# daigo0927/tf-raft

Hardware: NVIDIA H100
Metric: frame-pairs/sec at 448×512 iters=12; final-flow max-abs vs ref (higher is better)
Workload: dtype f32

## Files before the change

tf_raft_b200/csrc/conv_tc.cuh:

```cuda
#pragma once
#include "common.cuh"
#include "kernels.cuh"
#include "tmap.cuh"

namespace raft {

enum TcEpilogue : int {
  EPI_LINEAR = 0,
  EPI_GRU_ZR = 1,
  EPI_GRU_Q = 2,
};
enum TcAct : int { ACT_NONE = 0, ACT_RELU = 1 };

constexpr int kTileM = 128;
constexpr int kChunkK = 64;
constexpr int kABytes = kTileM * kChunkK * 2;
constexpr int kMaxTileN = 128;
constexpr int kConsumerWGs = 2;
constexpr int kConsumerWarps = 4 * kConsumerWGs;
constexpr int kTcThreads = 128 * kConsumerWGs + 128;
constexpr int kStageCols = 64;
constexpr int kStagingBytes = kConsumerWGs * 64 * kStageCols * 4;
constexpr int kSmemMax = 227 * 1024;
constexpr int kSmemFixed = 1024  + kStagingBytes + 512 ;

struct alignas(64) TcConvParams {
  CUtensorMap a_map[2];
  CUtensorMap b_map;
  int nseg, seg_chunks[2], seg_c0[2];
  int kh, kw, ph, pw;
  int stride;
  int B, H, W, TH, TW, tiles_x, tiles_y;
  int bn, n_total;
  int n_tiles_n;
  int nstages, stage_bytes;
  int group_chunks;
  int mode, act;
  const float* bias;
  const float* inv_scale;
  float out_scale;
  float* out_f32; int f32_stride, f32_c0;
  __half* out_hi; __half* out_lo; int h_stride, h_c0;
  const float* post_scale;
  const float* post_shift;
  const float* residual; int res_stride, res_c0;
  const float* concat_src; int concat_n;
  float* z; int hid;
  float* h;
  float* adv_coords;
  float* adv_flow;
};

#if defined(__CUDA_ARCH__)
__device__ __forceinline__ float4 ld4(const float* p) { return *reinterpret_cast<const float4*>(p); }
__device__ __forceinline__ float4 ldg4(const float* p) { return __ldg(reinterpret_cast<const float4*>(p)); }
__device__ __forceinline__ void st4(float* p, float4 v) { *reinterpret_cast<float4*>(p) = v; }
__device__ __forceinline__ void st8u(void* p, const uint32_t (&r)[8]) {
  reinterpret_cast<uint4*>(p)[0] = make_uint4(r[0], r[1], r[2], r[3]);
  reinterpret_cast<uint4*>(p)[1] = make_uint4(r[4], r[5], r[6], r[7]);
}
__device__ __forceinline__ void ldcg8(const float* p, float (&r)[8]) {
  const float4 a = __ldcg(reinterpret_cast<const float4*>(p)), b = __ldcg(reinterpret_cast<const float4*>(p) + 1);
  r[0] = a.x; r[1] = a.y; r[2] = a.z; r[3] = a.w; r[4] = b.x; r[5] = b.y; r[6] = b.z; r[7] = b.w;
}
__device__ __forceinline__ void ldnc8(const float* p, float (&r)[8]) {
  const float4 a = __ldg(reinterpret_cast<const float4*>(p)), b = __ldg(reinterpret_cast<const float4*>(p) + 1);
  r[0] = a.x; r[1] = a.y; r[2] = a.z; r[3] = a.w; r[4] = b.x; r[5] = b.y; r[6] = b.z; r[7] = b.w;
}
__device__ __forceinline__ void st8f(float* p, float a, float b, float c, float d, float e, float f, float g, float h) {
  const uint32_t r[8] = {__float_as_uint(a), __float_as_uint(b), __float_as_uint(c), __float_as_uint(d),
                         __float_as_uint(e), __float_as_uint(f), __float_as_uint(g), __float_as_uint(h)};
  st8u(p, r);
}
__device__ __forceinline__ float4 ldcg4(const float* p) { return __ldcg(reinterpret_cast<const float4*>(p)); }

__device__ __forceinline__ float fast_sigmoid(float x) { return __fdividef(1.0f, 1.0f + __expf(-x)); }
__device__ __forceinline__ float fast_tanh(float x) { return 1.0f - __fdividef(2.0f, 1.0f + __expf(2.0f * x)); }

template <int MODE>
__device__ __forceinline__ void tc_epilogue_regs(const TcConvParams& p, float (&v)[32], size_t pix, int col, int ncol,
                                                 float inv_scale) {
  if (p.bias) {
#pragma unroll
    for (int q = 0; q < 8; ++q) {
      const float4 bq = ldg4(p.bias + col + 4 * q);
      v[4 * q] = v[4 * q] * inv_scale + bq.x; v[4 * q + 1] = v[4 * q + 1] * inv_scale + bq.y;
      v[4 * q + 2] = v[4 * q + 2] * inv_scale + bq.z; v[4 * q + 3] = v[4 * q + 3] * inv_scale + bq.w;
    }
  } else {
#pragma unroll
    for (int j = 0; j < 32; ++j) v[j] *= inv_scale;
  }
  if (MODE == EPI_LINEAR && p.post_scale) {
#pragma unroll
    for (int q = 0; q < 8; ++q) {
      const float4 sc = ldg4(p.post_scale + col + 4 * q), sh = ldg4(p.post_shift + col + 4 * q);
      v[4 * q] = v[4 * q] * sc.x + sh.x; v[4 * q + 1] = v[4 * q + 1] * sc.y + sh.y;
      v[4 * q + 2] = v[4 * q + 2] * sc.z + sh.z; v[4 * q + 3] = v[4 * q + 3] * sc.w + sh.w;
    }
  }

  __half* dhi = nullptr;
  __half* dlo = nullptr;
  if (MODE == EPI_LINEAR) {
    const bool full = col + 32 <= p.n_total;
#pragma unroll
    for (int j = 0; j < 32; ++j) {
      if (p.act == ACT_RELU) v[j] = relu_nan(v[j]);
      v[j] *= p.out_scale;
    }
    if (full) {
      if (p.residual) {
        const float* rp = p.residual + pix * (size_t)p.res_stride + p.res_c0 + col;
        if (((p.res_stride | p.res_c0) & 7) == 0) {
#pragma unroll
          for (int q = 0; q < 4; ++q) {
            float r8[8];
            ldnc8(rp + 8 * q, r8);
#pragma unroll
            for (int e = 0; e < 8; ++e) v[8 * q + e] = relu_nan(v[8 * q + e] + r8[e]);
          }
        } else if (((p.res_stride | p.res_c0) & 3) == 0) {
#pragma unroll
          for (int q = 0; q < 8; ++q) {
            const float4 r4 = ldg4(rp + 4 * q);
            v[4 * q] = relu_nan(v[4 * q] + r4.x); v[4 * q + 1] = relu_nan(v[4 * q + 1] + r4.y);
            v[4 * q + 2] = relu_nan(v[4 * q + 2] + r4.z); v[4 * q + 3] = relu_nan(v[4 * q + 3] + r4.w);
          }
        } else {
#pragma unroll
          for (int j = 0; j < 32; ++j) v[j] = relu_nan(v[j] + __ldg(rp + j));
        }
      }
    } else {
#pragma unroll
      for (int j = 0; j < 32; ++j) {
        const int cj = col + j - p.n_total;
        if (cj >= 0) v[j] = (p.concat_src && cj < p.concat_n) ? __ldg(p.concat_src + pix * p.concat_n + cj) : 0.0f;
        else if (p.residual) v[j] = relu_nan(v[j] + __ldg(p.residual + pix * (size_t)p.res_stride + p.res_c0 + col + j));
      }
    }
    if (p.out_f32) {
      const int nvalid = min(ncol, p.n_total - col);
      float* dst = p.out_f32 + pix * (size_t)p.f32_stride + p.f32_c0 + col;
      if (nvalid == 32 && ((p.f32_stride | p.f32_c0) & 7) == 0) {
#pragma unroll
        for (int q = 0; q < 4; ++q)
          st8f(dst + 8 * q, v[8 * q], v[8 * q + 1], v[8 * q + 2], v[8 * q + 3], v[8 * q + 4], v[8 * q + 5], v[8 * q + 6], v[8 * q + 7]);
      } else if (nvalid == 32 && ((p.f32_stride | p.f32_c0) & 3) == 0) {
#pragma unroll
        for (int q = 0; q < 8; ++q) st4(dst + 4 * q, make_float4(v[4 * q], v[4 * q + 1], v[4 * q + 2], v[4 * q + 3]));
      } else {
#pragma unroll
        for (int j = 0; j < 32; ++j)
          if (j < nvalid) dst[j] = v[j];
      }
    }
    if (p.out_hi && ncol == 32) {
      const size_t o = pix * (size_t)p.h_stride + p.h_c0 + col;
      dhi = p.out_hi + o;
      dlo = p.out_lo + o;
    }
    if (p.adv_coords && col == 0) {
      float2 c1 = __ldcg(reinterpret_cast<const float2*>(p.adv_coords) + pix);
      c1.x = __fadd_rn(c1.x, v[0]);
      c1.y = __fadd_rn(c1.y, v[1]);
      reinterpret_cast<float2*>(p.adv_coords)[pix] = c1;
      const float gx = (float)(pix % p.W), gy = (float)((pix / p.W) % p.H);
      reinterpret_cast<float2*>(p.adv_flow)[pix] = make_float2(__fsub_rn(c1.x, gx), __fsub_rn(c1.y, gy));
    }
  } else if (MODE == EPI_GRU_ZR) {
    if (col < p.hid) {
      float* dst = p.z + pix * (size_t)p.hid + col;
      if ((p.hid & 7) == 0) {
#pragma unroll
        for (int q = 0; q < 4; ++q)
          st8f(dst + 8 * q, fast_sigmoid(v[8 * q]), fast_sigmoid(v[8 * q + 1]), fast_sigmoid(v[8 * q + 2]), fast_sigmoid(v[8 * q + 3]),
               fast_sigmoid(v[8 * q + 4]), fast_sigmoid(v[8 * q + 5]), fast_sigmoid(v[8 * q + 6]), fast_sigmoid(v[8 * q + 7]));
      } else {
#pragma unroll
        for (int q = 0; q < 8; ++q)
          st4(dst + 4 * q, make_float4(fast_sigmoid(v[4 * q]), fast_sigmoid(v[4 * q + 1]), fast_sigmoid(v[4 * q + 2]),
                                       fast_sigmoid(v[4 * q + 3])));
      }
    } else {
      const int hc = col - p.hid;
      const float* hp = p.h + pix * (size_t)p.hid + hc;
      if ((p.hid & 7) == 0) {
#pragma unroll
        for (int q = 0; q < 4; ++q) {
          float h8[8];
          ldcg8(hp + 8 * q, h8);
#pragma unroll
          for (int e = 0; e < 8; ++e) v[8 * q + e] = fast_sigmoid(v[8 * q + e]) * h8[e];
        }
      } else {
#pragma unroll
        for (int q = 0; q < 8; ++q) {
          const float4 hv = ldcg4(hp + 4 * q);
          v[4 * q] = fast_sigmoid(v[4 * q]) * hv.x; v[4 * q + 1] = fast_sigmoid(v[4 * q + 1]) * hv.y;
          v[4 * q + 2] = fast_sigmoid(v[4 * q + 2]) * hv.z; v[4 * q + 3] = fast_sigmoid(v[4 * q + 3]) * hv.w;
        }
      }
      const size_t o = pix * (size_t)p.h_stride + p.h_c0 + hc;
      dhi = p.out_hi + o;
      dlo = p.out_lo + o;
    }
  } else if (MODE == EPI_GRU_Q) {
    float* hrow = p.h + pix * (size_t)p.hid + col;
    const float* zp = p.z + pix * (size_t)p.hid + col;
#pragma unroll
    for (int q = 0; q < 8; ++q) {
      const float4 zv = ldcg4(zp + 4 * q), hv = ldcg4(hrow + 4 * q);
      v[4 * q] = (1.0f - zv.x) * hv.x + zv.x * fast_tanh(v[4 * q]);
      v[4 * q + 1] = (1.0f - zv.y) * hv.y + zv.y * fast_tanh(v[4 * q + 1]);
      v[4 * q + 2] = (1.0f - zv.z) * hv.z + zv.z * fast_tanh(v[4 * q + 2]);
      v[4 * q + 3] = (1.0f - zv.w) * hv.w + zv.w * fast_tanh(v[4 * q + 3]);
    }
#pragma unroll
    for (int q = 0; q < 8; ++q) st4(hrow + 4 * q, make_float4(v[4 * q], v[4 * q + 1], v[4 * q + 2], v[4 * q + 3]));
    const size_t o = pix * (size_t)p.h_stride + p.h_c0 + col;
    dhi = p.out_hi + o;
    dlo = p.out_lo + o;
  }

  if (dhi) {
    const bool wide = ((reinterpret_cast<uintptr_t>(dhi) | reinterpret_cast<uintptr_t>(dlo)) & 31) == 0;
#pragma unroll
    for (int q = 0; q < 2; ++q) {
      uint32_t ph[8], pl[8];
#pragma unroll
      for (int e = 0; e < 8; ++e) split_f16x2(v[16 * q + 2 * e], v[16 * q + 2 * e + 1], ph[e], pl[e]);
      if (wide) {
        st8u(dhi + 16 * q, ph);
        st8u(dlo + 16 * q, pl);
      } else {
        reinterpret_cast<uint4*>(dhi)[2 * q] = make_uint4(ph[0], ph[1], ph[2], ph[3]);
        reinterpret_cast<uint4*>(dhi)[2 * q + 1] = make_uint4(ph[4], ph[5], ph[6], ph[7]);
        reinterpret_cast<uint4*>(dlo)[2 * q] = make_uint4(pl[0], pl[1], pl[2], pl[3]);
        reinterpret_cast<uint4*>(dlo)[2 * q + 1] = make_uint4(pl[4], pl[5], pl[6], pl[7]);
      }
    }
  }
}

struct RingPos {
  int slot;
  uint32_t par;
};

__device__ __forceinline__ int ring_next(RingPos& r, int nst) {
  const int s = r.slot;
  r.slot = s + 1 == nst ? 0 : s + 1;
  return s;
}

__device__ __forceinline__ void ring_init(uint64_t* full_bar, uint64_t* empty_bar, int nst) {
  for (int s = 0; s < nst; ++s) {
    mbar_init(&full_bar[s], 1);
    mbar_init(&empty_bar[s], kConsumerWarps);
  }
}

struct RingSlot {
  uint8_t* data;
  uint64_t* full;
};

__device__ __forceinline__ RingSlot ring_acquire(uint8_t* stages, const int& slot_bytes, const int& nst, uint64_t* full_bar,
                                                 uint64_t* empty_bar, RingPos& rp, const int& tx) {
  const int s = ring_next(rp, nst);
  mbar_wait(&empty_bar[s], ((rp.par >> s) & 1u) ^ 1u);
  rp.par ^= 1u << s;
  mbar_arrive_expect_tx(&full_bar[s], (uint32_t)tx);
  return RingSlot{stages + (size_t)s * slot_bytes, &full_bar[s]};
}

template <int N>
__device__ __forceinline__ void ring_mma(float (&racc)[N / 2], uint8_t* stages, const int& slot_bytes, const int& nst,
                                         uint64_t* full_bar, uint64_t* empty_bar, RingPos& rp, int wg, uint32_t b_lo_off,
                                         int total, const int& group_chunks) {
  const int lane = threadIdx.x & 31;
  float acc[N / 2];
#pragma unroll
  for (int i = 0; i < N / 2; ++i) acc[i] = racc[i] = 0.0f;
  for (int done = 0; done < total;) {
    const int gend = min(total, done + group_chunks);
    for (int first = 1; done < gend; ++done, first = 0) {
      const int s = ring_next(rp, nst);
      mbar_wait(&full_bar[s], (rp.par >> s) & 1u);
      rp.par ^= 1u << s;
      const uint32_t sa = smem_u32(stages + (size_t)s * slot_bytes);
      const uint32_t arow = (uint32_t)wg * 64 * 128;
      wgmma_fence_regs(acc);
      wgmma_fence();
      wgmma_chunk3<N>(acc, make_desc_sw128(sa + arow), make_desc_sw128(sa + kABytes + arow), make_desc_sw128(sa + 2 * kABytes),
                      make_desc_sw128(sa + 2 * kABytes + b_lo_off), first != 0);
      wgmma_commit();
      wgmma_wait_all();
      wgmma_fence_regs(acc);
      __syncwarp();
      if (lane == 0) mbar_arrive(&empty_bar[s]);
    }
#pragma unroll
    for (int i = 0; i < N / 2; ++i) racc[i] += acc[i];
  }
}

__device__ __forceinline__ int tc_total_chunks(const TcConvParams& c) {
  return c.kh * c.kw * (c.seg_chunks[0] + (c.nseg > 1 ? c.seg_chunks[1] : 0));
}

__device__ __forceinline__ void tc_produce_tile(const TcConvParams& c, uint8_t* stages, uint64_t* full_bar, uint64_t* empty_bar,
                                                RingPos& rp, int nt, int b, int ty, int tx, unsigned int* next_item = nullptr,
                                                int* claim = nullptr) {
  const int ntaps = c.kh * c.kw;
  const int x0 = tx * c.TW * c.stride, y0 = ty * c.TH * c.stride, n0 = nt * c.bn;
  int left = tc_total_chunks(c);
  for (int tap = 0; tap < ntaps; ++tap) {
    const int dy = tap / c.kw - c.ph, dx = tap % c.kw - c.pw;
    int kc = 0;
    for (int seg = 0; seg < c.nseg; ++seg) {
      for (int ch = 0; ch < c.seg_chunks[seg]; ++ch, ++kc) {
        if (--left == 0 && claim) *claim = (int)atomicAdd(next_item, 1u);
        const RingSlot st = ring_acquire(stages, c.stage_bytes, c.nstages, full_bar, empty_bar, rp, c.stage_bytes);
        tma_load_5d(st.data, &c.a_map[seg], st.full, c.seg_c0[seg] + ch * kChunkK, x0 + dx, y0 + dy, b, 0);
        tma_load_4d(st.data + 2 * kABytes, &c.b_map, st.full, kc * kChunkK, n0, tap, 0);
      }
    }
  }
}

__device__ __forceinline__ int stg_idx(int r, int c) { return r * kStageCols + ((((c >> 2) ^ (r & 7))) << 2) + (c & 3); }

template <int N>
__device__ __forceinline__ void tc_consume_tile(const TcConvParams& c, uint8_t* stages, float* staging, uint64_t* full_bar,
                                                uint64_t* empty_bar, RingPos& rp, int wg, int tid, int nt, int b, int ty,
                                                int tx) {
  const int lane = tid & 31, w = tid >> 5;
  float racc[N / 2];
  ring_mma<N>(racc, stages, c.stage_bytes, c.nstages, full_bar, empty_bar, rp, wg, (uint32_t)(c.bn * kChunkK * 2),
              tc_total_chunks(c), c.group_chunks);

  float* stg = staging + wg * 64 * kStageCols;
  const int row = tid & 63, half = tid >> 6;
  const int m = wg * 64 + row;
  const int x = tx * c.TW + m % c.TW, y = ty * c.TH + m / c.TW;
  const bool inside = x < c.W && y < c.H;
  const size_t pix = ((size_t)b * c.H + y) * c.W + x;
  const float inv_scale = c.inv_scale ? __ldg(c.inv_scale) : 1.0f;
#pragma unroll
  for (int cb = 0; cb < (N + kStageCols - 1) / kStageCols; ++cb) {
    if (cb * kStageCols >= c.bn) break;
    wg_sync(wg);
#pragma unroll
    for (int i = cb * 8; i < min(cb * 8 + 8, N / 8); ++i) {
      const int col = 8 * (i - cb * 8) + 2 * (lane & 3), r0 = 16 * w + (lane >> 2);
      *reinterpret_cast<float2*>(stg + stg_idx(r0, col)) = make_float2(racc[4 * i], racc[4 * i + 1]);
      *reinterpret_cast<float2*>(stg + stg_idx(r0 + 8, col)) = make_float2(racc[4 * i + 2], racc[4 * i + 3]);
    }
    wg_sync(wg);
    const int c0 = cb * kStageCols + half * 32;
    if (inside && c0 < c.bn) {
      const int ncol = min(32, c.bn - c0);
      float v[32];
#pragma unroll
      for (int q = 0; q < 8; ++q) {
        const float4 t4 = *reinterpret_cast<const float4*>(stg + stg_idx(row, half * 32 + 4 * q));
        v[4 * q] = t4.x; v[4 * q + 1] = t4.y; v[4 * q + 2] = t4.z; v[4 * q + 3] = t4.w;
      }
#pragma unroll
      for (int j = 0; j < 32; ++j)
        if (j >= ncol) v[j] = 0.0f;
      if (c.mode == EPI_LINEAR) tc_epilogue_regs<EPI_LINEAR>(c, v, pix, nt * c.bn + c0, ncol, inv_scale);
      else if (c.mode == EPI_GRU_ZR) tc_epilogue_regs<EPI_GRU_ZR>(c, v, pix, nt * c.bn + c0, ncol, inv_scale);
      else tc_epilogue_regs<EPI_GRU_Q>(c, v, pix, nt * c.bn + c0, ncol, inv_scale);
    }
  }
}

template <class F>
__device__ __forceinline__ void with_mma_n(int bn, F&& f) {
  if (bn <= 16) f(std::integral_constant<int, 16>{});
  else if (bn <= 32) f(std::integral_constant<int, 32>{});
  else if (bn <= 64) f(std::integral_constant<int, 64>{});
  else if (bn <= 96) f(std::integral_constant<int, 96>{});
  else f(std::integral_constant<int, 128>{});
}

__device__ __forceinline__ void regs_producer() { asm volatile("setmaxnreg.dec.sync.aligned.u32 40;\n" ::: "memory"); }
__device__ __forceinline__ void regs_consumer() { asm volatile("setmaxnreg.inc.sync.aligned.u32 232;\n" ::: "memory"); }

__device__ __forceinline__ void tc_decode_tile(const TcConvParams& c, int t, int& nt, int& b, int& ty, int& tx) {
  const int mtiles = c.B * c.tiles_y * c.tiles_x;
  nt = t / mtiles;
  int mt = t - nt * mtiles;
  tx = mt % c.tiles_x;
  mt /= c.tiles_x;
  ty = mt % c.tiles_y;
  b = mt / c.tiles_y;
}
#endif

__global__ void __launch_bounds__(kTcThreads, 1) conv_tc_kernel(const __grid_constant__ TcConvParams p) {
#if defined(__CUDA_ARCH__)
  extern __shared__ uint8_t smem_raw[];
  uint8_t* smem = reinterpret_cast<uint8_t*>((reinterpret_cast<uintptr_t>(smem_raw) + 1023) & ~uintptr_t(1023));
  const int nst = p.nstages;
  uint8_t* stages = smem;
  float* staging = reinterpret_cast<float*>(stages + (size_t)nst * p.stage_bytes);
  uint64_t* full_bar = reinterpret_cast<uint64_t*>(reinterpret_cast<uint8_t*>(staging) + kStagingBytes);
  uint64_t* empty_bar = full_bar + nst;

  const int warp = threadIdx.x >> 5;
  const int mtiles = p.B * p.tiles_y * p.tiles_x;
  const int ntiles = mtiles * p.n_tiles_n;

  if (threadIdx.x == 0) {
    ring_init(full_bar, empty_bar, nst);
    fence_mbar_init();
  }
  if (warp == kConsumerWarps && (threadIdx.x & 31) == 0) {
    prefetch_tmap(&p.a_map[0]);
    prefetch_tmap(&p.b_map);
    if (p.nseg > 1) prefetch_tmap(&p.a_map[1]);
  }
  __syncthreads();
  asm volatile("griddepcontrol.wait;" ::: "memory");
  asm volatile("griddepcontrol.launch_dependents;" ::: "memory");

  RingPos rp{0, 0u};
  if (warp >= kConsumerWarps) {
    regs_producer();
    if (warp == kConsumerWarps && elect_one()) {
      for (int t = blockIdx.x; t < ntiles; t += gridDim.x) {
        int nt, b, ty, tx;
        tc_decode_tile(p, t, nt, b, ty, tx);
        tc_produce_tile(p, stages, full_bar, empty_bar, rp, nt, b, ty, tx);
      }
    }
  } else {
    regs_consumer();
    const int wg = warp >> 2, tid = threadIdx.x & 127;
    with_mma_n(p.bn, [&](auto n) {
      for (int t = blockIdx.x; t < ntiles; t += gridDim.x) {
        int nt, b, ty, tx;
        tc_decode_tile(p, t, nt, b, ty, tx);
        tc_consume_tile<decltype(n)::value>(p, stages, staging, full_bar, empty_bar, rp, wg, tid, nt, b, ty, tx);
      }
    });
  }
#endif
}

inline void tc_pick_tile(int W, int H, int* tw, int* th) {
  long best = -1;
  for (int t = 128; t >= 8; t >>= 1) {
    const int hh = 128 / t;
    const long area = (long)round_up(W, t) * round_up(H, hh);
    if (best < 0 || area < best) {
      best = area;
      *tw = t;
      *th = hh;
    }
  }
}

inline int tc_n_split(int bn) {
  const int f = ceil_div(bn, kMaxTileN);
  return bn % (16 * f) == 0 ? f : 0;
}

inline int tc_finalize(TcConvParams& p) {
  p.tiles_x = ceil_div(p.W, p.TW);
  p.tiles_y = ceil_div(p.H, p.TH);
  p.stage_bytes = 2 * kABytes + 2 * p.bn * kChunkK * 2;
  int nst = (kSmemMax - kSmemFixed) / p.stage_bytes;
  if (nst > 8) nst = 8;
  p.nstages = nst;
  return nst * p.stage_bytes + kSmemFixed;
}

inline int tc_check(const TcConvParams& p) {
  if (p.bn % 16 != 0 || p.bn < 16 || p.bn > kMaxTileN || p.TW * p.TH != kTileM) return RAFT_ERR_BAD_SHAPE;
  if (p.mode != EPI_LINEAR && p.mode != EPI_GRU_ZR && p.mode != EPI_GRU_Q) return RAFT_ERR_UNSUPPORTED;
  if (p.group_chunks < 1) return RAFT_ERR_BAD_ARG;
  return RAFT_OK;
}

template <auto Kernel>
inline int persistent_grid(int smem, long items, unsigned* grid) {
  static int num_sms[64] = {0};
  int dev = 0;
  RAFT_CUDA_TRY(cudaGetDevice(&dev));
  int& sms = num_sms[dev & 63];
  if (!sms) {
    RAFT_CUDA_TRY(cudaFuncSetAttribute(Kernel, cudaFuncAttributeMaxDynamicSharedMemorySize, smem));
    RAFT_CUDA_TRY(cudaDeviceGetAttribute(&sms, cudaDevAttrMultiProcessorCount, dev));
  }
  *grid = (unsigned)(items < sms ? items : sms);
  return RAFT_OK;
}

inline int tc_launch(TcConvParams& p, int n_tiles_n, cudaStream_t stream) {
  RAFT_TRY(tc_check(p));
  if (p.stride < 1) p.stride = 1;
  const int smem = tc_finalize(p);
  if (p.nstages < 2) return RAFT_ERR_UNSUPPORTED;
  p.n_tiles_n = n_tiles_n;
  unsigned grid = 0;
  RAFT_TRY(persistent_grid<conv_tc_kernel>(kSmemMax, (long)p.B * p.tiles_y * p.tiles_x * n_tiles_n, &grid));
  cudaLaunchConfig_t cfg;
  memset(&cfg, 0, sizeof(cfg));
  cfg.gridDim = dim3(grid);
  cfg.blockDim = dim3((unsigned)kTcThreads);
  cfg.dynamicSmemBytes = (size_t)smem;
  cfg.stream = stream;
  cudaLaunchAttribute attr[1];
  attr[0].id = cudaLaunchAttributeProgrammaticStreamSerialization;
  attr[0].val.programmaticStreamSerializationAllowed = 1;
  cfg.attrs = attr;
  cfg.numAttrs = 1;
  ++g_launches;
  RAFT_CUDA_TRY(cudaLaunchKernelEx(&cfg, conv_tc_kernel, p));
  return raft_launch_status();
}

struct TcWeightSlot {
  size_t hi, lo, bias, scale, absmax;
  int kh, kw, cin_pad, cout_pad;
};

inline TcWeightSlot tc_weight_slot(size_t& off, int kh, int kw, int cin_pad, int cout_pad) {
  auto take = [&](size_t bytes) { const size_t o = off; off = align_up(off + bytes, 256); return o; };
  TcWeightSlot s;
  s.kh = kh; s.kw = kw; s.cin_pad = cin_pad; s.cout_pad = cout_pad;
  const size_t plane = (size_t)kh * kw * cout_pad * cin_pad * sizeof(__half);
  s.hi = take(plane);
  s.lo = take(plane);
  s.bias = take(sizeof(float) * (cout_pad + 64));
  s.scale = take(2 * sizeof(float));
  s.absmax = take(sizeof(unsigned int));
  return s;
}

struct TcCinMap { int nrange, src0[2], n[2], dst0[2]; };

inline int tc_pack_weights(uint8_t* base, const TcWeightSlot& s, const raft_conv* const src[], int nsrc,
                           const TcCinMap* cin_map, bool flatten, cudaStream_t st) {
  unsigned int* amax = reinterpret_cast<unsigned int*>(base + s.absmax);
  float* scale = reinterpret_cast<float*>(base + s.scale);
  for (int i = 0; i < nsrc; ++i) {
    const size_t nw = (size_t)src[i]->kh * src[i]->kw * src[i]->cin * src[i]->cout;
    RAFT_TRY(launch(absmax_kernel, grid_for(nw), 256, 0, st, src[i]->kernel, nw, amax));
  }
  RAFT_TRY(launch(weight_scale_kernel, 1, 1, 0, st, amax, scale));
  int cout_off = 0;
  for (int i = 0; i < nsrc; ++i) {
    const raft_conv& cv = *src[i];
    PackParams pp;
    memset(&pp, 0, sizeof(pp));
    pp.w = cv.kernel;
    pp.kh = cv.kh; pp.kw = cv.kw; pp.cin = cv.cin; pp.cout = cv.cout;
    if (flatten) { pp.cin = pp.kh * pp.kw * pp.cin; pp.kh = pp.kw = 1; }
    pp.hi = reinterpret_cast<__half*>(base + s.hi);
    pp.lo = reinterpret_cast<__half*>(base + s.lo);
    pp.cout_pad = s.cout_pad; pp.cin_pad = s.cin_pad; pp.cout_off = cout_off;
    const TcCinMap m = cin_map ? *cin_map : TcCinMap{1, {0, 0}, {pp.cin, 0}, {0, 0}};
    pp.nrange = m.nrange;
    for (int r = 0; r < m.nrange; ++r) {
      pp.r_src0[r] = m.src0[r];
      pp.r_n[r] = m.n[r];
      pp.r_dst0[r] = m.dst0[r];
    }
    pp.scale = scale;
    RAFT_TRY(launch(pack_weights_kernel, grid_for((size_t)cv.kh * cv.kw * cv.cin * cv.cout), 256, 0, st, pp));
    RAFT_CUDA_TRY(cudaMemcpyAsync(base + s.bias + cout_off * sizeof(float), cv.bias, cv.cout * sizeof(float),
                                  cudaMemcpyDeviceToDevice, st));
    cout_off += cv.cout;
  }
  return RAFT_OK;
}

inline int tc_use_weights(TcConvParams& p, const uint8_t* base, const TcWeightSlot& s, int bn) {
  RAFT_TRY(make_tmap_wgt2(&p.b_map, reinterpret_cast<const __half*>(base + s.hi),
                          reinterpret_cast<const __half*>(base + s.lo), s.kh * s.kw, s.cout_pad, s.cin_pad, bn));
  p.kh = s.kh; p.kw = s.kw;
  p.bn = bn;
  p.bias = reinterpret_cast<const float*>(base + s.bias);
  p.inv_scale = reinterpret_cast<const float*>(base + s.scale) + 1;
  return RAFT_OK;
}

}
```

tf_raft_b200/csrc/encoder.cuh:

```cuda
#pragma once
#include <algorithm>

#include "lookup.cuh"
#include "update.cuh"

namespace raft {

enum { NORM_NONE = 0, NORM_INSTANCE = 1, NORM_BATCH = 2 };

struct EncSpec { int c0; int c[3]; int s[3]; };
inline EncSpec enc_spec(int variant) {
  if (variant == RAFT_VARIANT_BASIC) return {64, {64, 96, 128}, {1, 2, 2}};
  return {32, {32, 64, 96}, {1, 2, 2}};
}
inline int pad64(int c) { return round_up(c, 64); }

struct EncNormSlot { size_t gamma, beta, fscale, fshift; int C; };
struct EncLayout {
  TcWeightSlot conv1;
  EncNormSlot norm1;
  TcWeightSlot bc1[6], bc2[6], bds[6];
  EncNormSlot bn1[6], bn2[6], bnd[6];
  int has_ds[6], bc[6], bstride[6];
  TcWeightSlot conv2;
  size_t total;
};

inline EncLayout enc_layout(int variant, int out_dim) {
  EncLayout L;
  memset(&L, 0, sizeof(L));
  const EncSpec S = enc_spec(variant);
  size_t off = 0;
  auto take = [&](size_t bytes) { size_t o = off; off = align_up(off + bytes, 256); return o; };
  auto conv_slot = [&](int kh, int kw, int cin, int cout) { return tc_weight_slot(off, kh, kw, pad64(cin), round_up(cout, 32)); };
  auto norm_slot = [&](int C) {
    EncNormSlot n;
    n.C = C;
    n.gamma = take(sizeof(float) * (C + 64)); n.beta = take(sizeof(float) * (C + 64));
    n.fscale = take(sizeof(float) * (C + 64)); n.fshift = take(sizeof(float) * (C + 64));
    return n;
  };
  L.conv1 = conv_slot(1, 1, 147, S.c0);
  L.norm1 = norm_slot(S.c0);
  int cin = S.c0;
  for (int k = 0; k < 6; ++k) {
    const int c = S.c[k / 2], st = (k % 2 == 0) ? S.s[k / 2] : 1;
    L.bc[k] = c; L.bstride[k] = st;
    L.bc1[k] = conv_slot(3, 3, cin, c);
    L.bc2[k] = conv_slot(3, 3, c, c);
    L.bn1[k] = norm_slot(c);
    L.bn2[k] = norm_slot(c);
    L.has_ds[k] = st != 1;
    if (L.has_ds[k]) { L.bds[k] = conv_slot(1, 1, cin, c); L.bnd[k] = norm_slot(c); }
    cin = c;
  }
  L.conv2 = conv_slot(1, 1, cin, out_dim);
  L.total = off;
  return L;
}

struct EncWs {
  float *X32, *O32, *Y32, *D32;
  __half *Xh, *Xl, *Oh, *Ol, *Fh, *Fl, *Ih, *Il;
  float *part, *mean, *mult;
  size_t total;
};
constexpr int kNormSplit = 64;
inline EncWs enc_ws_layout(void* base, int variant, int N, int H, int W) {
  EncWs E;
  memset(&E, 0, sizeof(E));
  const EncSpec S = enc_spec(variant);
  size_t max32 = 0, max16 = 0;
  for (int l = 0; l < 3; ++l) {
    const int d = 2 << l;
    const size_t np = (size_t)N * ((H + d - 1) / d) * ((W + d - 1) / d);
    const int c = l == 0 ? (S.c0 > S.c[0] ? S.c0 : S.c[0]) : S.c[l];
    if (np * c > max32) max32 = np * c;
    if (np * pad64(c) > max16) max16 = np * pad64(c);
  }
  uint8_t* b8 = reinterpret_cast<uint8_t*>(base);
  size_t off = 0;
  auto take = [&](size_t bytes) { uint8_t* p = b8 + off; off = align_up(off + bytes, 1024); return p; };
  E.X32 = (float*)take(max32 * 4); E.O32 = (float*)take(max32 * 4);
  E.Y32 = (float*)take(max32 * 4); E.D32 = (float*)take(max32 * 4);
  E.Xh = (__half*)take(max16 * 2); E.Xl = (__half*)take(max16 * 2);
  E.Oh = (__half*)take(max16 * 2); E.Ol = (__half*)take(max16 * 2);
  E.Fh = (__half*)take(max16 * 2); E.Fl = (__half*)take(max16 * 2);
  {
    const size_t np1 = (size_t)N * ((H + 1) / 2) * ((W + 1) / 2);
    E.Ih = (__half*)take(np1 * 192 * 2); E.Il = (__half*)take(np1 * 192 * 2);
  }
  E.part = (float*)take((size_t)N * kNormSplit * 3 * 256 * 4);
  E.mean = (float*)take((size_t)N * 256 * 4);
  E.mult = (float*)take((size_t)N * 256 * 4);
  E.total = off;
  return E;
}

inline int enc_pack_conv(const raft_conv& cv, int kh, int kw, int cin, int cout, const TcWeightSlot& s, bool flatten,
                         uint8_t* base, cudaStream_t st) {
  if (!cv.kernel || !cv.bias) return RAFT_ERR_BAD_ARG;
  if (cv.kh != kh || cv.kw != kw || cv.cin != cin || cv.cout != cout) return RAFT_ERR_BAD_SHAPE;
  const raft_conv* src[1] = {&cv};
  return tc_pack_weights(base, s, src, 1, nullptr, flatten, st);
}

inline int enc_pack_norm(const raft_norm& nm, const EncNormSlot& s, int norm_type, uint8_t* base, cudaStream_t st) {
  if (norm_type == NORM_NONE) return 0;
  if (!nm.gamma || !nm.beta) return RAFT_ERR_BAD_ARG;
  float* g = reinterpret_cast<float*>(base + s.gamma);
  float* b = reinterpret_cast<float*>(base + s.beta);
  RAFT_CUDA_TRY(cudaMemcpyAsync(g, nm.gamma, s.C * sizeof(float), cudaMemcpyDeviceToDevice, st));
  RAFT_CUDA_TRY(cudaMemcpyAsync(b, nm.beta, s.C * sizeof(float), cudaMemcpyDeviceToDevice, st));
  if (norm_type == NORM_BATCH) {
    if (!nm.moving_mean || !nm.moving_variance) return RAFT_ERR_BAD_ARG;
    return launch(bn_fold_kernel, ceil_div(s.C, 128), 128, 0, st, nm.gamma, nm.beta, nm.moving_mean, nm.moving_variance,
                  1e-3f, s.C, reinterpret_cast<float*>(base + s.fscale), reinterpret_cast<float*>(base + s.fshift));
  }
  return raft_launch_status();
}

inline int encoder_prepare(int variant, int norm_type, int out_dim, const raft_encoder_weights* w, void* prepared,
                           size_t bytes, cudaStream_t st) {
  const EncLayout L = enc_layout(variant, out_dim);
  if (L.total > bytes) return RAFT_ERR_WORKSPACE;
  const EncSpec S = enc_spec(variant);
  uint8_t* base = reinterpret_cast<uint8_t*>(prepared);
  RAFT_CUDA_TRY(cudaMemsetAsync(base, 0, L.total, st));
  RAFT_TRY(enc_pack_conv(w->conv1, 7, 7, 3, S.c0, L.conv1, true, base, st));
  RAFT_TRY(enc_pack_norm(w->norm1, L.norm1, norm_type, base, st));
  int cin = S.c0;
  for (int k = 0; k < 6; ++k) {
    const int c = L.bc[k];
    RAFT_TRY(enc_pack_conv(w->block[k].conv1, 3, 3, cin, c, L.bc1[k], false, base, st));
    RAFT_TRY(enc_pack_conv(w->block[k].conv2, 3, 3, c, c, L.bc2[k], false, base, st));
    RAFT_TRY(enc_pack_norm(w->block[k].norm1, L.bn1[k], norm_type, base, st));
    RAFT_TRY(enc_pack_norm(w->block[k].norm2, L.bn2[k], norm_type, base, st));
    if (L.has_ds[k]) {
      RAFT_TRY(enc_pack_conv(w->block[k].downsample, 1, 1, cin, c, L.bds[k], false, base, st));
      RAFT_TRY(enc_pack_norm(w->block[k].downsample_norm, L.bnd[k], norm_type, base, st));
    }
    cin = c;
  }
  RAFT_TRY(enc_pack_conv(w->conv2, 1, 1, cin, out_dim, L.conv2, false, base, st));
  return raft_launch_status();
}

struct EncCtx {
  const uint8_t* prep; EncLayout L; EncWs W; cudaStream_t st;
  int N, norm_type, stats;
  int per_image;
};

inline int enc_norm_apply(const EncCtx& c, const EncNormSlot& ns, const float* y, size_t npix, int P, int relu,
                          const float* skip32, const __half* skip_hi, const __half* skip_lo, float* out32, __half* hi,
                          __half* lo) {
  const int C = ns.C, G = c.per_image ? c.N : 1;
  const int Pg = c.per_image ? P : (int)npix;
  const float* gamma = reinterpret_cast<const float*>(c.prep + ns.gamma);
  const float* beta = reinterpret_cast<const float*>(c.prep + ns.beta);
  RAFT_TRY(launch(norm_stats_kernel, dim3((unsigned)G, kNormSplit), 256, 0, c.st, y, Pg, C, kNormSplit, c.W.part));
  RAFT_TRY(launch(norm_final_kernel, ceil_div(G * C * 32, 256), 256, 0, c.st, c.W.part, G, C, kNormSplit, gamma, 1e-3f,
                  c.W.mean, c.W.mult));
  return launch(norm_apply_kernel, grid_for(npix * (pad64(C) / 8)), 256, 0, c.st, y, npix, P, C, c.per_image, c.W.mean,
                c.W.mult, beta, relu, skip32, skip_hi, skip_lo, out32, hi, lo, pad64(C));
}

inline int enc_conv_tc(const EncCtx& c, const TcWeightSlot& cs, int cout, const EncNormSlot* ns, const __half* ahi,
                       const __half* alo, int Hin, int Win, int Hout, int Wout, int stride, int relu, const float* skip,
                       float* out32, __half* ohi, __half* olo) {
  TcConvParams p;
  memset(&p, 0, sizeof(p));
  int tw, th;
  tc_pick_tile(Wout, Hout, &tw, &th);
  if (tw * stride > 256) tw = 128 / stride, th = 128 / tw;
  const int nsplit = tc_n_split(cs.cout_pad);
  if (!nsplit) return RAFT_ERR_BAD_SHAPE;
  RAFT_TRY(make_tmap_act2(&p.a_map[0], ahi, alo, c.N, Hin, Win, cs.cin_pad, tw, th, stride));
  RAFT_TRY(tc_use_weights(p, c.prep, cs, cs.cout_pad / nsplit));
  p.nseg = 1; p.seg_chunks[0] = cs.cin_pad / kChunkK; p.seg_c0[0] = 0;
  p.stride = stride;
  if (stride == 1) { p.ph = (cs.kh - 1) / 2; p.pw = (cs.kw - 1) / 2; }
  else {
    const int tot_h = (Hout - 1) * stride + cs.kh - Hin, tot_w = (Wout - 1) * stride + cs.kw - Win;
    p.ph = (tot_h > 0 ? tot_h : 0) / 2; p.pw = (tot_w > 0 ? tot_w : 0) / 2;
  }
  p.B = c.N; p.H = Hout; p.W = Wout; p.TH = th; p.TW = tw;
  p.n_total = cout;
  p.mode = EPI_LINEAR; p.out_scale = 1.0f;
  p.out_f32 = out32; p.f32_stride = cout; p.f32_c0 = 0;
  p.out_hi = ohi; p.out_lo = olo; p.h_stride = pad64(cout); p.h_c0 = 0;
  if (ns && !c.stats && c.norm_type == NORM_BATCH) {
    p.post_scale = reinterpret_cast<const float*>(c.prep + ns->fscale);
    p.post_shift = reinterpret_cast<const float*>(c.prep + ns->fshift);
  }
  const bool fused = !(ns && c.stats);
  if (fused) {
    p.act = relu ? ACT_RELU : ACT_NONE;
    p.residual = skip; p.res_stride = cout; p.res_c0 = 0;
  } else {
    p.act = ACT_NONE; p.out_hi = nullptr; p.out_lo = nullptr;
  }
  p.group_chunks = 5;
  return tc_launch(p, nsplit, c.st);
}

inline int encoder_forward(int variant, int norm_type, int out_dim, const void* prepared, const float* images, int N,
                           int H, int W, int training, int image_norm, float* out, void* ws, size_t ws_bytes, cudaStream_t st) {
  EncCtx c;
  c.prep = reinterpret_cast<const uint8_t*>(prepared);
  c.L = enc_layout(variant, out_dim);
  c.W = enc_ws_layout(ws, variant, N, H, W);
  if (c.W.total > ws_bytes) return RAFT_ERR_WORKSPACE;
  c.st = st; c.N = N; c.norm_type = norm_type;
  c.stats = (norm_type == NORM_INSTANCE) || (norm_type == NORM_BATCH && training);
  c.per_image = norm_type == NORM_INSTANCE;
  const EncSpec S = enc_spec(variant);
  const EncLayout& L = c.L;
  const EncWs& E = c.W;

  int h = (H + 1) / 2, w = (W + 1) / 2;
  {
    const size_t npix = (size_t)N * h * w;
    const int tot_h = (h - 1) * 2 + 7 - H, tot_w = (w - 1) * 2 + 7 - W;
    const float* src = images;
    if (image_norm) {
      const size_t nimg = (size_t)N * H * W * 3;
      RAFT_TRY(launch(image_norm_kernel, grid_for(nimg), 256, 0, st, images, E.O32, nimg));
      src = E.O32;
    }
    RAFT_TRY(launch(stem_im2col_kernel, grid_for(npix * 24), 256, 0, st, src, N, H, W, h, w, (tot_h > 0 ? tot_h : 0) / 2,
                    (tot_w > 0 ? tot_w : 0) / 2, 0, E.Ih, E.Il));
    if (!c.stats && pad64(S.c0) != S.c0) {
      RAFT_CUDA_TRY(cudaMemsetAsync(E.Xh, 0, npix * pad64(S.c0) * 2, st));
      RAFT_CUDA_TRY(cudaMemsetAsync(E.Xl, 0, npix * pad64(S.c0) * 2, st));
    }
    RAFT_TRY(enc_conv_tc(c, L.conv1, S.c0, &L.norm1, E.Ih, E.Il, h, w, h, w, 1, 1, nullptr, c.stats ? E.Y32 : E.X32, E.Xh, E.Xl));
    if (c.stats) RAFT_TRY(enc_norm_apply(c, L.norm1, E.Y32, npix, h * w, 1, nullptr, nullptr, nullptr, nullptr, E.Xh, E.Xl));
  }

  float *X32 = E.X32, *O32 = E.O32;
  __half *Xh = E.Xh, *Xl = E.Xl, *Oh = E.Oh, *Ol = E.Ol;
  for (int k = 0; k < 6; ++k) {
    const int st2 = L.bstride[k], cc = L.bc[k];
    const int ho = (h + st2 - 1) / st2, wo = (w + st2 - 1) / st2;
    const size_t npo = (size_t)N * ho * wo;
    const bool zero_pad_out = pad64(cc) != cc;
    if (!c.stats && zero_pad_out) {
      RAFT_CUDA_TRY(cudaMemsetAsync(E.Fh, 0, npo * pad64(cc) * 2, st));
      RAFT_CUDA_TRY(cudaMemsetAsync(E.Fl, 0, npo * pad64(cc) * 2, st));
      RAFT_CUDA_TRY(cudaMemsetAsync(Oh, 0, npo * pad64(cc) * 2, st));
      RAFT_CUDA_TRY(cudaMemsetAsync(Ol, 0, npo * pad64(cc) * 2, st));
    }
    RAFT_TRY(enc_conv_tc(c, L.bc1[k], cc, &L.bn1[k], Xh, Xl, h, w, ho, wo, st2, 1, nullptr, c.stats ? E.Y32 : nullptr, E.Fh, E.Fl));
    if (c.stats) RAFT_TRY(enc_norm_apply(c, L.bn1[k], E.Y32, npo, ho * wo, 1, nullptr, nullptr, nullptr, nullptr, E.Fh, E.Fl));
    const float* skip = X32;
    if (L.has_ds[k]) {
      RAFT_TRY(enc_conv_tc(c, L.bds[k], cc, &L.bnd[k], Xh, Xl, h, w, ho, wo, st2, 0, nullptr, c.stats ? E.Y32 : E.D32, nullptr, nullptr));
      if (c.stats) RAFT_TRY(enc_norm_apply(c, L.bnd[k], E.Y32, npo, ho * wo, 0, nullptr, nullptr, nullptr, E.D32, nullptr, nullptr));
      skip = E.D32;
    }
    RAFT_TRY(enc_conv_tc(c, L.bc2[k], cc, &L.bn2[k], E.Fh, E.Fl, ho, wo, ho, wo, 1, 1, skip, c.stats ? E.Y32 : O32, Oh, Ol));
    if (c.stats) {
      if (L.has_ds[k]) RAFT_TRY(enc_norm_apply(c, L.bn2[k], E.Y32, npo, ho * wo, 1, E.D32, nullptr, nullptr, nullptr, Oh, Ol));
      else RAFT_TRY(enc_norm_apply(c, L.bn2[k], E.Y32, npo, ho * wo, 1, nullptr, Xh, Xl, nullptr, Oh, Ol));
    }
    float* t32 = X32; X32 = O32; O32 = t32;
    __half* th_ = Xh; Xh = Oh; Oh = th_;
    __half* tl_ = Xl; Xl = Ol; Ol = tl_;
    h = ho; w = wo;
  }
  RAFT_TRY(enc_conv_tc(c, L.conv2, out_dim, nullptr, Xh, Xl, h, w, h, w, 1, 0, nullptr, out, nullptr, nullptr));
  return raft_launch_status();
}

}
```

Before: 311.2.

## Add halo-tile TMA path for 3x3 stride-1 64-channel encoder convs

For 3x3 stride-1 convolutions with 64 input channels and a 128x1 pixel tile, the producer loads one 130-wide activation row strip per kernel row, plus the three tap weights, into a single stage. The consumer reuses that strip for all three horizontal taps by shifting the shared-memory descriptor one row per tap, rather than issuing a separate A-tile TMA per tap. This cuts activation load traffic and ring stages for these encoder layers. The trade-offs are larger stages (so fewer of them), a wgmma wait after every tap, and descriptor offsets that do not line up with 128B-swizzle atom boundaries, which could hurt correctness or bank behaviour.

```diff
diff --git a/tf_raft_b200/csrc/conv_tc.cuh b/tf_raft_b200/csrc/conv_tc.cuh
--- a/tf_raft_b200/csrc/conv_tc.cuh
+++ b/tf_raft_b200/csrc/conv_tc.cuh
@@ -23,6 +23,9 @@
 constexpr int kStagingBytes = kConsumerWGs * 64 * kStageCols * 4;
 constexpr int kSmemMax = 227 * 1024;
 constexpr int kSmemFixed = 1024  + kStagingBytes + 512 ;
+constexpr int kHaloW = kTileM + 2;
+constexpr int kHaloABox = 2 * kHaloW * kChunkK * 2;
+constexpr int kHaloABytes = (kHaloABox + 1023) / 1024 * 1024;
 
 struct alignas(64) TcConvParams {
   CUtensorMap a_map[2];
@@ -49,6 +52,7 @@
   float* h;
   float* adv_coords;
   float* adv_flow;
+  int halo;
 };
 
 #if defined(__CUDA_ARCH__)
@@ -331,16 +335,64 @@
   }
 }
 
+__device__ __forceinline__ void tc_produce_tile_halo(const TcConvParams& c, uint8_t* stages, uint64_t* full_bar,
+                                                     uint64_t* empty_bar, RingPos& rp, int nt, int b, int ty, int tx) {
+  const int wbytes = c.bn * kChunkK * 2 * 2;
+  const int tx_bytes = kHaloABox + 3 * wbytes;
+  for (int dy = 0; dy < 3; ++dy) {
+    const RingSlot st = ring_acquire(stages, c.stage_bytes, c.nstages, full_bar, empty_bar, rp, tx_bytes);
+    tma_load_5d(st.data, &c.a_map[0], st.full, 0, tx * kTileM - 1, ty + dy - 1, b, 0);
+    for (int dx = 0; dx < 3; ++dx)
+      tma_load_4d(st.data + kHaloABytes + dx * wbytes, &c.b_map, st.full, 0, nt * c.bn, dy * 3 + dx, 0);
+  }
+}
+
+template <int N>
+__device__ __forceinline__ void ring_mma_halo(float (&racc)[N / 2], uint8_t* stages, const TcConvParams& c, uint64_t* full_bar,
+                                              uint64_t* empty_bar, RingPos& rp, int wg) {
+  const int lane = threadIdx.x & 31;
+  const uint32_t wbytes = (uint32_t)(c.bn * kChunkK * 2 * 2), b_lo_off = wbytes / 2;
+  float acc[N / 2];
+#pragma unroll
+  for (int i = 0; i < N / 2; ++i) acc[i] = racc[i] = 0.0f;
+  int k = 0;
+  for (int dy = 0; dy < 3; ++dy) {
+    const int s = ring_next(rp, c.nstages);
+    mbar_wait(&full_bar[s], (rp.par >> s) & 1u);
+    rp.par ^= 1u << s;
+    const uint32_t sa = smem_u32(stages + (size_t)s * c.stage_bytes);
+    for (int dx = 0; dx < 3; ++dx, ++k) {
+      const uint32_t a = sa + (uint32_t)(wg * 64 + dx) * 128, bw = sa + kHaloABytes + dx * wbytes;
+      wgmma_fence_regs(acc);
+      wgmma_fence();
+      wgmma_chunk3<N>(acc, make_desc_sw128(a), make_desc_sw128(a + kHaloW * 128), make_desc_sw128(bw),
+                      make_desc_sw128(bw + b_lo_off), k % c.group_chunks == 0);
+      wgmma_commit();
+      wgmma_wait_all();
+      wgmma_fence_regs(acc);
+      if ((k + 1) % c.group_chunks == 0 || k == 8) {
+#pragma unroll
+        for (int i = 0; i < N / 2; ++i) racc[i] += acc[i];
+      }
+    }
+    __syncwarp();
+    if (lane == 0) mbar_arrive(&empty_bar[s]);
+  }
+}
+
 __device__ __forceinline__ int stg_idx(int r, int c) { return r * kStageCols + ((((c >> 2) ^ (r & 7))) << 2) + (c & 3); }
 
-template <int N>
+template <int N, bool HALO = false>
 __device__ __forceinline__ void tc_consume_tile(const TcConvParams& c, uint8_t* stages, float* staging, uint64_t* full_bar,
                                                 uint64_t* empty_bar, RingPos& rp, int wg, int tid, int nt, int b, int ty,
                                                 int tx) {
   const int lane = tid & 31, w = tid >> 5;
   float racc[N / 2];
-  ring_mma<N>(racc, stages, c.stage_bytes, c.nstages, full_bar, empty_bar, rp, wg, (uint32_t)(c.bn * kChunkK * 2),
-              tc_total_chunks(c), c.group_chunks);
+  if constexpr (HALO)
+    ring_mma_halo<N>(racc, stages, c, full_bar, empty_bar, rp, wg);
+  else
+    ring_mma<N>(racc, stages, c.stage_bytes, c.nstages, full_bar, empty_bar, rp, wg, (uint32_t)(c.bn * kChunkK * 2),
+                tc_total_chunks(c), c.group_chunks);
 
   float* stg = staging + wg * 64 * kStageCols;
   const int row = tid & 63, half = tid >> 6;
@@ -436,7 +488,8 @@
       for (int t = blockIdx.x; t < ntiles; t += gridDim.x) {
         int nt, b, ty, tx;
         tc_decode_tile(p, t, nt, b, ty, tx);
-        tc_produce_tile(p, stages, full_bar, empty_bar, rp, nt, b, ty, tx);
+        if (p.halo) tc_produce_tile_halo(p, stages, full_bar, empty_bar, rp, nt, b, ty, tx);
+        else tc_produce_tile(p, stages, full_bar, empty_bar, rp, nt, b, ty, tx);
       }
     }
   } else {
@@ -446,7 +499,8 @@
       for (int t = blockIdx.x; t < ntiles; t += gridDim.x) {
         int nt, b, ty, tx;
         tc_decode_tile(p, t, nt, b, ty, tx);
-        tc_consume_tile<decltype(n)::value>(p, stages, staging, full_bar, empty_bar, rp, wg, tid, nt, b, ty, tx);
+        if (p.halo) tc_consume_tile<decltype(n)::value, true>(p, stages, staging, full_bar, empty_bar, rp, wg, tid, nt, b, ty, tx);
+        else tc_consume_tile<decltype(n)::value>(p, stages, staging, full_bar, empty_bar, rp, wg, tid, nt, b, ty, tx);
       }
     });
   }
@@ -474,7 +528,7 @@
 inline int tc_finalize(TcConvParams& p) {
   p.tiles_x = ceil_div(p.W, p.TW);
   p.tiles_y = ceil_div(p.H, p.TH);
-  p.stage_bytes = 2 * kABytes + 2 * p.bn * kChunkK * 2;
+  p.stage_bytes = p.halo ? kHaloABytes + 3 * 2 * p.bn * kChunkK * 2 : 2 * kABytes + 2 * p.bn * kChunkK * 2;
   int nst = (kSmemMax - kSmemFixed) / p.stage_bytes;
   if (nst > 8) nst = 8;
   p.nstages = nst;
@@ -485,6 +539,9 @@
   if (p.bn % 16 != 0 || p.bn < 16 || p.bn > kMaxTileN || p.TW * p.TH != kTileM) return RAFT_ERR_BAD_SHAPE;
   if (p.mode != EPI_LINEAR && p.mode != EPI_GRU_ZR && p.mode != EPI_GRU_Q) return RAFT_ERR_UNSUPPORTED;
   if (p.group_chunks < 1) return RAFT_ERR_BAD_ARG;
+  if (p.halo && (p.kh != 3 || p.kw != 3 || p.ph != 1 || p.pw != 1 || p.stride != 1 || p.nseg != 1 || p.seg_chunks[0] != 1 ||
+                 p.TW != kTileM || p.TH != 1))
+    return RAFT_ERR_UNSUPPORTED;
   return RAFT_OK;
 }
 
diff --git a/tf_raft_b200/csrc/encoder.cuh b/tf_raft_b200/csrc/encoder.cuh
--- a/tf_raft_b200/csrc/encoder.cuh
+++ b/tf_raft_b200/csrc/encoder.cuh
@@ -176,7 +176,9 @@
   if (tw * stride > 256) tw = 128 / stride, th = 128 / tw;
   const int nsplit = tc_n_split(cs.cout_pad);
   if (!nsplit) return RAFT_ERR_BAD_SHAPE;
-  RAFT_TRY(make_tmap_act2(&p.a_map[0], ahi, alo, c.N, Hin, Win, cs.cin_pad, tw, th, stride));
+  p.halo = cs.kh == 3 && cs.kw == 3 && stride == 1 && cs.cin_pad == kChunkK && tw == kTileM && th == 1 &&
+           cs.cout_pad <= 64;
+  RAFT_TRY(make_tmap_act2(&p.a_map[0], ahi, alo, c.N, Hin, Win, cs.cin_pad, p.halo ? kHaloW : tw, th, stride));
   RAFT_TRY(tc_use_weights(p, c.prep, cs, cs.cout_pad / nsplit));
   p.nseg = 1; p.seg_chunks[0] = cs.cin_pad / kChunkK; p.seg_c0[0] = 0;
   p.stride = stride;
```

New measurement: 313.0, median of 6. About the same (+0.6%).
